# lucidrains/magvit2-pytorch

Hardware: NVIDIA H100
Metric: video-frames/sec tokenize+decode, 17x128x128 bf16 (higher is better)
Workload: dtype bf16

## Files before the change

magvit2_pytorch_b200/csrc/tc_common.cuh:

```cuda
#pragma once
#include "common.cuh"
#include <cuda.h>
#include <mutex>

namespace mv2 {


__device__ __forceinline__ uint32_t smem_u32(const void* p) { return (uint32_t)__cvta_generic_to_shared(p); }

__device__ __forceinline__ void mbar_init(uint32_t bar, uint32_t count) {
  asm volatile("mbarrier.init.shared::cta.b64 [%0], %1;" ::"r"(bar), "r"(count));
}
__device__ __forceinline__ void mbar_expect_tx(uint32_t bar, uint32_t bytes) {
  asm volatile("mbarrier.arrive.expect_tx.shared::cta.b64 _, [%0], %1;" ::"r"(bar), "r"(bytes) : "memory");
}
__device__ __forceinline__ void mbar_wait(uint32_t bar, uint32_t parity) {
  asm volatile(
      "{\n\t"
      ".reg .pred P1;\n\t"
      "WAIT_LOOP:\n\t"
      "mbarrier.try_wait.parity.shared::cta.b64 P1, [%0], %1, 0x989680;\n\t"
      "@P1 bra DONE;\n\t"
      "bra WAIT_LOOP;\n\t"
      "DONE:\n\t"
      "}" ::"r"(bar), "r"(parity) : "memory");
}
__device__ __forceinline__ void fence_barrier_init() { asm volatile("fence.mbarrier_init.release.cluster;" ::: "memory"); }
__device__ __forceinline__ void fence_proxy_async() { asm volatile("fence.proxy.async.shared::cta;" ::: "memory"); }

__device__ __forceinline__ void tma_load_5d(uint32_t dst, const CUtensorMap* map, uint32_t bar, int c0, int c1, int c2,
                                            int c3, int c4) {
  asm volatile(
      "cp.async.bulk.tensor.5d.shared::cluster.global.tile.mbarrier::complete_tx::bytes [%0], [%1, {%3, %4, %5, %6, %7}], [%2];"
      ::"r"(dst), "l"(map), "r"(bar), "r"(c0), "r"(c1), "r"(c2), "r"(c3), "r"(c4) : "memory");
}
__device__ __forceinline__ void tma_load_2d(uint32_t dst, const CUtensorMap* map, uint32_t bar, int c0, int c1) {
  asm volatile(
      "cp.async.bulk.tensor.2d.shared::cluster.global.tile.mbarrier::complete_tx::bytes [%0], [%1, {%3, %4}], [%2];"
      ::"r"(dst), "l"(map), "r"(bar), "r"(c0), "r"(c1) : "memory");
}
__device__ __forceinline__ void tma_load_3d(uint32_t dst, const CUtensorMap* map, uint32_t bar, int c0, int c1, int c2) {
  asm volatile(
      "cp.async.bulk.tensor.3d.shared::cluster.global.tile.mbarrier::complete_tx::bytes [%0], [%1, {%3, %4, %5}], [%2];"
      ::"r"(dst), "l"(map), "r"(bar), "r"(c0), "r"(c1), "r"(c2) : "memory");
}
__device__ __forceinline__ void tma_prefetch_desc(const CUtensorMap* map) {
  asm volatile("prefetch.tensormap [%0];" ::"l"(map) : "memory");
}

__device__ __forceinline__ void wgmma_fence() { asm volatile("wgmma.fence.sync.aligned;" ::: "memory"); }
__device__ __forceinline__ void wgmma_commit() { asm volatile("wgmma.commit_group.sync.aligned;" ::: "memory"); }
__device__ __forceinline__ void wgmma_wait_all() { asm volatile("wgmma.wait_group.sync.aligned 0;" ::: "memory"); }
template <int N> __device__ __forceinline__ void wgmma_wait() { asm volatile("wgmma.wait_group.sync.aligned %0;" ::"n"(N) : "memory"); }

template <int N> __device__ __forceinline__ void setmaxnreg_dec() { asm volatile("setmaxnreg.dec.sync.aligned.u32 %0;" ::"n"(N)); }
template <int N> __device__ __forceinline__ void setmaxnreg_inc() { asm volatile("setmaxnreg.inc.sync.aligned.u32 %0;" ::"n"(N)); }
template <int N> __device__ __forceinline__ void wgmma_bf16(float (&d)[N / 2], uint64_t da, uint64_t db, uint32_t scale_d);
template <> __device__ __forceinline__ void wgmma_bf16<8>(float (&d)[4], uint64_t da, uint64_t db, uint32_t scale_d) {
  asm volatile(
      "{\n\t.reg .pred p;\n\tsetp.ne.b32 p, %6, 0;\n\t"
      "wgmma.mma_async.sync.aligned.m64n8k16.f32.bf16.bf16 {%0, %1, %2, %3}, %4, %5, p, 1, 1, 0, 0;\n\t}"
      : "+f"(d[0]), "+f"(d[1]), "+f"(d[2]), "+f"(d[3])
      : "l"(da), "l"(db), "r"(scale_d));
}
template <> __device__ __forceinline__ void wgmma_bf16<16>(float (&d)[8], uint64_t da, uint64_t db, uint32_t scale_d) {
  asm volatile(
      "{\n\t.reg .pred p;\n\tsetp.ne.b32 p, %10, 0;\n\t"
      "wgmma.mma_async.sync.aligned.m64n16k16.f32.bf16.bf16 {%0, %1, %2, %3, %4, %5, %6, %7}, %8, %9, p, 1, 1, 0, 0;\n\t}"
      : "+f"(d[0]), "+f"(d[1]), "+f"(d[2]), "+f"(d[3]), "+f"(d[4]), "+f"(d[5]), "+f"(d[6]), "+f"(d[7])
      : "l"(da), "l"(db), "r"(scale_d));
}
template <> __device__ __forceinline__ void wgmma_bf16<32>(float (&d)[16], uint64_t da, uint64_t db, uint32_t scale_d) {
  asm volatile(
      "{\n\t.reg .pred p;\n\tsetp.ne.b32 p, %18, 0;\n\t"
      "wgmma.mma_async.sync.aligned.m64n32k16.f32.bf16.bf16 {%0, %1, %2, %3, %4, %5, %6, %7, %8, %9, %10, %11, %12, %13, %14, %15}, %16, %17, p, 1, 1, 0, 0;\n\t}"
      : "+f"(d[0]), "+f"(d[1]), "+f"(d[2]), "+f"(d[3]), "+f"(d[4]), "+f"(d[5]), "+f"(d[6]), "+f"(d[7]), "+f"(d[8]), "+f"(d[9]), "+f"(d[10]), "+f"(d[11]), "+f"(d[12]), "+f"(d[13]), "+f"(d[14]), "+f"(d[15])
      : "l"(da), "l"(db), "r"(scale_d));
}
template <> __device__ __forceinline__ void wgmma_bf16<64>(float (&d)[32], uint64_t da, uint64_t db, uint32_t scale_d) {
  asm volatile(
      "{\n\t.reg .pred p;\n\tsetp.ne.b32 p, %34, 0;\n\t"
      "wgmma.mma_async.sync.aligned.m64n64k16.f32.bf16.bf16 {%0, %1, %2, %3, %4, %5, %6, %7, %8, %9, %10, %11, %12, %13, %14, %15, %16, %17, %18, %19, %20, %21, %22, %23, %24, %25, %26, %27, %28, %29, %30, %31}, %32, %33, p, 1, 1, 0, 0;\n\t}"
      : "+f"(d[0]), "+f"(d[1]), "+f"(d[2]), "+f"(d[3]), "+f"(d[4]), "+f"(d[5]), "+f"(d[6]), "+f"(d[7]), "+f"(d[8]), "+f"(d[9]), "+f"(d[10]), "+f"(d[11]), "+f"(d[12]), "+f"(d[13]), "+f"(d[14]), "+f"(d[15]), "+f"(d[16]), "+f"(d[17]), "+f"(d[18]), "+f"(d[19]), "+f"(d[20]), "+f"(d[21]), "+f"(d[22]), "+f"(d[23]), "+f"(d[24]), "+f"(d[25]), "+f"(d[26]), "+f"(d[27]), "+f"(d[28]), "+f"(d[29]), "+f"(d[30]), "+f"(d[31])
      : "l"(da), "l"(db), "r"(scale_d));
}
template <> __device__ __forceinline__ void wgmma_bf16<128>(float (&d)[64], uint64_t da, uint64_t db, uint32_t scale_d) {
  asm volatile(
      "{\n\t.reg .pred p;\n\tsetp.ne.b32 p, %66, 0;\n\t"
      "wgmma.mma_async.sync.aligned.m64n128k16.f32.bf16.bf16 {%0, %1, %2, %3, %4, %5, %6, %7, %8, %9, %10, %11, %12, %13, %14, %15, %16, %17, %18, %19, %20, %21, %22, %23, %24, %25, %26, %27, %28, %29, %30, %31, %32, %33, %34, %35, %36, %37, %38, %39, %40, %41, %42, %43, %44, %45, %46, %47, %48, %49, %50, %51, %52, %53, %54, %55, %56, %57, %58, %59, %60, %61, %62, %63}, %64, %65, p, 1, 1, 0, 0;\n\t}"
      : "+f"(d[0]), "+f"(d[1]), "+f"(d[2]), "+f"(d[3]), "+f"(d[4]), "+f"(d[5]), "+f"(d[6]), "+f"(d[7]), "+f"(d[8]), "+f"(d[9]), "+f"(d[10]), "+f"(d[11]), "+f"(d[12]), "+f"(d[13]), "+f"(d[14]), "+f"(d[15]), "+f"(d[16]), "+f"(d[17]), "+f"(d[18]), "+f"(d[19]), "+f"(d[20]), "+f"(d[21]), "+f"(d[22]), "+f"(d[23]), "+f"(d[24]), "+f"(d[25]), "+f"(d[26]), "+f"(d[27]), "+f"(d[28]), "+f"(d[29]), "+f"(d[30]), "+f"(d[31]), "+f"(d[32]), "+f"(d[33]), "+f"(d[34]), "+f"(d[35]), "+f"(d[36]), "+f"(d[37]), "+f"(d[38]), "+f"(d[39]), "+f"(d[40]), "+f"(d[41]), "+f"(d[42]), "+f"(d[43]), "+f"(d[44]), "+f"(d[45]), "+f"(d[46]), "+f"(d[47]), "+f"(d[48]), "+f"(d[49]), "+f"(d[50]), "+f"(d[51]), "+f"(d[52]), "+f"(d[53]), "+f"(d[54]), "+f"(d[55]), "+f"(d[56]), "+f"(d[57]), "+f"(d[58]), "+f"(d[59]), "+f"(d[60]), "+f"(d[61]), "+f"(d[62]), "+f"(d[63])
      : "l"(da), "l"(db), "r"(scale_d));
}

__host__ __device__ __forceinline__ uint64_t gmma_desc_hi(uint32_t sbo, uint32_t row_bytes) {
  const uint64_t layout = row_bytes == 128 ? 1 : (row_bytes == 64 ? 2 : 3);
  return ((uint64_t)1 << 16) | ((uint64_t)(sbo >> 4) << 32) | (layout << 62);
}
__device__ __forceinline__ uint32_t desc_lo(uint32_t saddr) { return (saddr & 0x3FFFF) >> 4; }

template <int N> __device__ __forceinline__ void stage_acc(const float (&d)[N / 2], float* stg, int t) {
  const int r = 16 * (t >> 5) + ((t & 31) >> 2), c = 2 * (t & 3);
#pragma unroll
  for (int j = 0; j < N / 8; ++j) {
    *reinterpret_cast<float2*>(stg + r * (N + 4) + 8 * j + c) = make_float2(d[4 * j], d[4 * j + 1]);
    *reinterpret_cast<float2*>(stg + (r + 8) * (N + 4) + 8 * j + c) = make_float2(d[4 * j + 2], d[4 * j + 3]);
  }
}
__device__ __forceinline__ void load_row32(const float* src, int ncols, uint32_t (&r)[32]) {
#pragma unroll
  for (int g = 0; g < 8; ++g) {
    if (g * 4 >= ncols) break;
    const float4 v = *reinterpret_cast<const float4*>(src + 4 * g);
    r[4 * g] = __float_as_uint(v.x); r[4 * g + 1] = __float_as_uint(v.y);
    r[4 * g + 2] = __float_as_uint(v.z); r[4 * g + 3] = __float_as_uint(v.w);
  }
}
__device__ __forceinline__ void named_bar_sync(uint32_t id, uint32_t nthreads) {
  asm volatile("bar.sync %0, %1;" ::"r"(id), "r"(nthreads) : "memory");
}
__device__ __forceinline__ void mbar_arrive(uint32_t bar) {
  asm volatile("mbarrier.arrive.shared::cta.b64 _, [%0];" ::"r"(bar) : "memory");
}

__device__ __forceinline__ uint32_t pack_bf16x2(float a, float b) {
  __nv_bfloat162 v = __floats2bfloat162_rn(a, b);
  return *reinterpret_cast<uint32_t*>(&v);
}



struct TcEpi {
  const float* bias;
  const __nv_bfloat16* res;
  __nv_bfloat16* y;
  int act, shuffle, mode;
  int Co;
  int To, Ho, Wo;
  int out_cf;
  const float* oscale;
};

__device__ __forceinline__ void store8_bf16(__nv_bfloat16* dst, const float (&v)[8]) {
  uint4 o;
  o.x = pack_bf16x2(v[0], v[1]); o.y = pack_bf16x2(v[2], v[3]);
  o.z = pack_bf16x2(v[4], v[5]); o.w = pack_bf16x2(v[6], v[7]);
  *reinterpret_cast<uint4*>(dst) = o;
}

enum { EPI_PLAIN = 0, EPI_GEGLU = 1, EPI_SHUFFLE = 2, EPI_RAGGED = 3, EPI_PLAIN_RES = 4, EPI_FUSED_RU = 5, EPI_SHUFFLE_ST = 6,
       EPI_DOWN_SPACE = 7 };

__device__ __forceinline__ float ex2_approx(float x) {
  float y;
  asm("ex2.approx.ftz.f32 %0, %1;" : "=f"(y) : "f"(x));
  return y;
}
__device__ __forceinline__ float rcp_approx(float x) {
  float y;
  asm("rcp.approx.ftz.f32 %0, %1;" : "=f"(y) : "f"(x));
  return y;
}
__device__ __forceinline__ float erf_fast(float x) {
  const float ax = fabsf(x);
  const float t = rcp_approx(fmaf(0.3275911f, ax, 1.f));
  float p = fmaf(1.061405429f, t, -1.453152027f);
  p = fmaf(p, t, 1.421413741f);
  p = fmaf(p, t, -0.284496736f);
  p = fmaf(p, t, 0.254829592f);
  const float e = ex2_approx(-1.4426950408889634f * ax * ax);
  return copysignf(fmaf(-p * t, e, 1.f), x);
}

__device__ __forceinline__ float gelu_fast(float g) {
  const float ag = fabsf(g);
  const float t = rcp_approx(fmaf(0.3275911f * 0.70710678118654752440f, ag, 1.f));
  float p = fmaf(0.5f * 1.061405429f, t, 0.5f * -1.453152027f);
  p = fmaf(p, t, 0.5f * 1.421413741f);
  p = fmaf(p, t, 0.5f * -0.284496736f);
  p = fmaf(p, t, 0.5f * 0.254829592f);
  const float e = ex2_approx((g * g) * (-0.5f * 1.4426950408889634f));
  const float q = (p * t) * e;
  return fmaf(-ag, q, fmaxf(g, 0.f));
}

template <int ACT>
__device__ __forceinline__ float act_ct(float x, bool relu = false) {
  if (ACT == MV2_ACT_ELU) {
    const float e = ex2_approx(x * 1.4426950408889634f) - 1.f;
    return x > 0.f ? x : e;
  }
  if (ACT == MV2_ACT_SILU) return x * rcp_approx(1.f + ex2_approx(-1.4426950408889634f * x));
  if (ACT == MV2_ACT_LEAKY_RELU) return x > 0.f ? x : (relu ? 0.f * x : 0.1f * x);
  return x;
}

template <int MODE, int ACT>
__device__ __forceinline__ void epi_chunk32_t(const TcEpi& e, const uint32_t (&r)[32], int ncols, int n, const float* sb,
                                              int b, int to, int ho, int wo, int64_t row_base, bool relu = false) {
  if (MODE == EPI_GEGLU) {
    const int I = e.Co >> 1;
    const int64_t pos = (((int64_t)b * e.To + to) * e.Ho + ho) * e.Wo + wo;
#pragma unroll
    for (int g = 0; g < 2; ++g) {
      if (g * 16 >= ncols || n + g * 16 >= e.Co) break;
      float v[8];
#pragma unroll
      for (int q = 0; q < 8; ++q) {
        const float xv = __uint_as_float(r[g * 16 + q]) + sb[g * 16 + q];
        const float gt = __uint_as_float(r[g * 16 + 8 + q]) + sb[g * 16 + 8 + q];
        v[q] = gelu_fast(gt) * xv;
      }
      store8_bf16(e.y + pos * I + ((n + g * 16) >> 1), v);
    }
    return;
  }
  const int cy = MODE == EPI_SHUFFLE ? (e.shuffle == MV2_SHUFFLE_SPACE ? (e.Co >> 2) : (e.Co >> 1)) : e.Co;
  const bool vec_ok = (cy & 7) == 0;
#pragma unroll
  for (int g = 0; g < 4; ++g) {
    const int ng = n + g * 8;
    if (g * 8 >= ncols || ng >= e.Co) break;
    float v[8];
    {
      const float4 b0 = *reinterpret_cast<const float4*>(sb + g * 8), b1 = *reinterpret_cast<const float4*>(sb + g * 8 + 4);
      const float bb[8] = {b0.x, b0.y, b0.z, b0.w, b1.x, b1.y, b1.z, b1.w};
      if (MODE != EPI_SHUFFLE && e.oscale) {
#pragma unroll
        for (int q = 0; q < 8; ++q) {
          const float os = ng + q < e.Co ? e.oscale[(int64_t)b * e.Co + ng + q] : 0.f;
          v[q] = act_ct<ACT>(__uint_as_float(r[g * 8 + q]) * os + bb[q], relu);
        }
      } else
#pragma unroll
      for (int q = 0; q < 8; ++q) v[q] = act_ct<ACT>(__uint_as_float(r[g * 8 + q]) + bb[q], relu);
    }
    int64_t off;
    if (MODE == EPI_SHUFFLE) {
      const int qd = ng / cy, c = ng - qd * cy;
      if (e.shuffle == MV2_SHUFFLE_SPACE) {
        const int p1 = qd >> 1, p2 = qd & 1;
        off = ((((int64_t)b * e.To + to) * (2 * e.Ho) + (2 * ho + p1)) * (2 * e.Wo) + (2 * wo + p2)) * cy + c;
      } else {
        off = ((((int64_t)b * (2 * e.To) + (2 * to + qd)) * e.Ho + ho) * e.Wo + wo) * cy + c;
      }
    } else {
      off = row_base + ng;
    }
    const float rscale = e.mode == 2 ? 0.70710678118654752440f : 1.f;
    if (vec_ok && ng + 8 <= e.Co) {
      if (e.res) {
        const uint4 rv = *reinterpret_cast<const uint4*>(e.res + off);
        const __nv_bfloat162* rb = reinterpret_cast<const __nv_bfloat162*>(&rv);
#pragma unroll
        for (int q = 0; q < 4; ++q) {
          const float2 f = __bfloat1622float2(rb[q]);
          v[2 * q] = (v[2 * q] + f.x) * rscale;
          v[2 * q + 1] = (v[2 * q + 1] + f.y) * rscale;
        }
      }
      store8_bf16(e.y + off, v);
    } else {
      if (MODE == EPI_RAGGED && e.out_cf) {
        const int64_t plane = (int64_t)e.Ho * e.Wo;
        const int64_t o0 = ((int64_t)b * e.Co * e.To + to) * plane + (int64_t)ho * e.Wo + wo;
        for (int q = 0; q < 8 && ng + q < e.Co; ++q) e.y[o0 + (int64_t)(ng + q) * e.To * plane] = __float2bfloat16_rn(v[q]);
      } else
      for (int q = 0; q < 8 && ng + q < e.Co; ++q) {
        float x = v[q];
        if (e.res) x = (x + __bfloat162float(e.res[off + q])) * rscale;
        e.y[off + q] = __float2bfloat16_rn(x);
      }
    }
  }
}

template <int ACT>
__device__ __forceinline__ void epi_pack32_t(const uint32_t (&r)[32], const float* sb, uint32_t (&pk)[16], bool relu = false) {
#pragma unroll
  for (int g = 0; g < 8; ++g) {
    const float4 b = *reinterpret_cast<const float4*>(sb + g * 4);
    pk[2 * g] = pack_bf16x2(act_ct<ACT>(__uint_as_float(r[4 * g]) + b.x, relu), act_ct<ACT>(__uint_as_float(r[4 * g + 1]) + b.y, relu));
    pk[2 * g + 1] = pack_bf16x2(act_ct<ACT>(__uint_as_float(r[4 * g + 2]) + b.z, relu), act_ct<ACT>(__uint_as_float(r[4 * g + 3]) + b.w, relu));
  }
}
template <int ACT>
__device__ __forceinline__ void epi_act32_t(uint32_t (&r)[32], const float* sb, bool relu = false) {
#pragma unroll
  for (int g = 0; g < 8; ++g) {
    const float4 b = *reinterpret_cast<const float4*>(sb + g * 4);
    r[4 * g] = __float_as_uint(act_ct<ACT>(__uint_as_float(r[4 * g]) + b.x, relu));
    r[4 * g + 1] = __float_as_uint(act_ct<ACT>(__uint_as_float(r[4 * g + 1]) + b.y, relu));
    r[4 * g + 2] = __float_as_uint(act_ct<ACT>(__uint_as_float(r[4 * g + 2]) + b.z, relu));
    r[4 * g + 3] = __float_as_uint(act_ct<ACT>(__uint_as_float(r[4 * g + 3]) + b.w, relu));
  }
}
__device__ __forceinline__ void epi_act32(int act, uint32_t (&r)[32], const float* sb) {
  if (act == MV2_ACT_ELU) epi_act32_t<MV2_ACT_ELU>(r, sb);
  else if (act == MV2_ACT_SILU) epi_act32_t<MV2_ACT_SILU>(r, sb);
  else if (act == MV2_ACT_LEAKY_RELU || act == MV2_ACT_RELU) epi_act32_t<MV2_ACT_LEAKY_RELU>(r, sb, act == MV2_ACT_RELU);
  else epi_act32_t<MV2_ACT_NONE>(r, sb);
}
__device__ __forceinline__ void epi_pack32(int act, const uint32_t (&r)[32], const float* sb, uint32_t (&pk)[16]) {
  if (act == MV2_ACT_ELU) epi_pack32_t<MV2_ACT_ELU>(r, sb, pk);
  else if (act == MV2_ACT_SILU) epi_pack32_t<MV2_ACT_SILU>(r, sb, pk);
  else if (act == MV2_ACT_LEAKY_RELU || act == MV2_ACT_RELU) epi_pack32_t<MV2_ACT_LEAKY_RELU>(r, sb, pk, act == MV2_ACT_RELU);
  else epi_pack32_t<MV2_ACT_NONE>(r, sb, pk);
}

template <int MODE>
__device__ __forceinline__ void epi_chunk32(const TcEpi& e, const uint32_t (&r)[32], int ncols, int n, const float* sb,
                                            int b, int to, int ho, int wo, int64_t row_base) {
  if (MODE == EPI_GEGLU) { epi_chunk32_t<EPI_GEGLU, MV2_ACT_NONE>(e, r, ncols, n, sb, b, to, ho, wo, row_base); return; }
  if (e.act == MV2_ACT_ELU) epi_chunk32_t<MODE, MV2_ACT_ELU>(e, r, ncols, n, sb, b, to, ho, wo, row_base);
  else if (e.act == MV2_ACT_SILU) epi_chunk32_t<MODE, MV2_ACT_SILU>(e, r, ncols, n, sb, b, to, ho, wo, row_base);
  else if (e.act == MV2_ACT_LEAKY_RELU || e.act == MV2_ACT_RELU)
    epi_chunk32_t<MODE, MV2_ACT_LEAKY_RELU>(e, r, ncols, n, sb, b, to, ho, wo, row_base, e.act == MV2_ACT_RELU);
  else epi_chunk32_t<MODE, MV2_ACT_NONE>(e, r, ncols, n, sb, b, to, ho, wo, row_base);
}

typedef CUresult (*EncodeTiledFn)(CUtensorMap*, CUtensorMapDataType, cuuint32_t, void*, const cuuint64_t*,
                                  const cuuint64_t*, const cuuint32_t*, const cuuint32_t*, CUtensorMapInterleave,
                                  CUtensorMapSwizzle, CUtensorMapL2promotion, CUtensorMapFloatOOBfill);

static inline EncodeTiledFn get_encode_fn() {
  static EncodeTiledFn fn = nullptr;
  static std::once_flag once;
  std::call_once(once, [] {
    void* f = nullptr;
    cudaDriverEntryPointQueryResult q;
    if (cudaGetDriverEntryPoint("cuTensorMapEncodeTiled", &f, cudaEnableDefault, &q) == cudaSuccess &&
        q == cudaDriverEntryPointSuccess)
      fn = (EncodeTiledFn)f;
  });
  return fn;
}

static inline CUtensorMapSwizzle swizzle_of_row(int row_bytes) {
  return row_bytes == 128 ? CU_TENSOR_MAP_SWIZZLE_128B : (row_bytes == 64 ? CU_TENSOR_MAP_SWIZZLE_64B : CU_TENSOR_MAP_SWIZZLE_32B);
}

static inline int encode_bf16_map(CUtensorMap* map, int rank, const void* base, const cuuint64_t* dims,
                                  const cuuint64_t* strides, const cuuint32_t* box, CUtensorMapSwizzle swz, const char* what) {
  const EncodeTiledFn enc = get_encode_fn();
  if (!enc) { set_error("cuTensorMapEncodeTiled entry point unavailable"); return MV2_E_CUDA; }
  const cuuint32_t es[5] = {1, 1, 1, 1, 1};
  const CUresult r = enc(map, CU_TENSOR_MAP_DATA_TYPE_BFLOAT16, (cuuint32_t)rank, const_cast<void*>(base), dims, strides, box, es,
                         CU_TENSOR_MAP_INTERLEAVE_NONE, swz, CU_TENSOR_MAP_L2_PROMOTION_L2_256B, CU_TENSOR_MAP_FLOAT_OOB_FILL_NONE);
  if (r != CUDA_SUCCESS) { set_error("cuTensorMapEncodeTiled(%s) failed: %d", what, (int)r); return MV2_E_CUDA; }
  return MV2_OK;
}

static inline TcEpi tc_epi_of(const mv2_tc_conv_args* a) {
  TcEpi e = {};
  e.bias = a->bias; e.res = (const __nv_bfloat16*)a->res; e.y = (__nv_bfloat16*)a->y;
  e.act = a->act; e.shuffle = a->shuffle; e.mode = a->epi_mode; e.Co = a->Co;
  e.To = a->To; e.Ho = a->Ho; e.Wo = a->Wo; e.out_cf = a->out_layout == 1; e.oscale = a->oscale;
  return e;
}

static inline int pow2_ceil(int v) { int r = 1; while (r < v) r <<= 1; return r; }
static inline int floor_div(int a, int b) { int q = a / b; if ((a % b != 0) && ((a < 0) != (b < 0))) --q; return q; }


}
```

magvit2_pytorch_b200/csrc/tc_slab.cu:

```cuda
#include "common.cuh"
#include "tc_common.cuh"
#include <cuda.h>
#include <algorithm>
#include <type_traits>
#include <mutex>
#include <map>
#include <vector>
#include <string.h>

namespace mv2 {

struct alignas(64) SlabParams {
  CUtensorMap amap;
  CUtensorMap hmap;
  CUtensorMap wmap;
  CUtensorMap wmap2;
  int kt, kh, kw, pt, ph, pw;
  int st;
  int hist_T;
  int Ci, kchunks, row_bytes;
  int B, T, H, W, Co;
  int mw, pitch, slab_h, slab_bytes, slab_stride;
  int bn, n_tiles_n, tiles_w, tiles_h, total_tiles;
  int slab_stages, w_stages;
  int tpw;
  TcEpi epi;
  CUtensorMap w1map;
  const float* bias1;
  const float* se_wk;
  float se_bk;
  float* se_ws;
  CUtensorMap amap_odd;
  int dn_e_off;
  int dn_aoff[6];
  int dn_lower;
  int h_stride;
};

__host__ __device__ __forceinline__ void slab_frame_of(const SlabParams& p, int slot, int& b, int& t) {
  const int ptc = p.pt > 0 ? (p.pt + p.st - 1) / p.st : 0;
  const int n_cheap = ptc < p.T ? ptc : p.T, n_full = p.T - n_cheap;
  const int full_slots = p.B * n_full;
  if (slot < full_slots) { b = slot / n_full; t = n_cheap + slot - b * n_full; }
  else { const int r = slot - full_slots; const int level = r / p.B; b = r - level * p.B; t = n_cheap - 1 - level; }
}
__host__ __device__ __forceinline__ int slab_tile_of_cta(const SlabParams& p, int k, int cta, int grid) {
  const int tile = k * grid + ((k & 1) ? grid - 1 - cta : cta);
  return tile < p.total_tiles ? tile : -1;
}
__device__ __forceinline__ int slab_tile_of(const SlabParams& p, int k) { return slab_tile_of_cta(p, k, blockIdx.x, gridDim.x); }

struct TileCoord { int b, t, h0, w0, n0; };
__host__ __device__ __forceinline__ TileCoord decode_tile(const SlabParams& p, int tile) {
  TileCoord c;
  const int nt = tile % p.n_tiles_n; tile /= p.n_tiles_n;
  const int tw = tile % p.tiles_w; tile /= p.tiles_w;
  const int th = tile % p.tiles_h; tile /= p.tiles_h;
  slab_frame_of(p, tile, c.b, c.t);
  c.h0 = th * 16;
  c.w0 = tw * 8 * p.mw;
  c.n0 = nt * p.bn;
  return c;
}

struct SlabSmem { uint32_t sbias, stage0, lpart, accstg, hbuf, end; };
__host__ __device__ __forceinline__ SlabSmem slab_smem_layout(const SlabParams& p, uint32_t bar0, bool fused) {
  SlabSmem m;
  m.sbias = (bar0 + 8 * (2 * p.slab_stages + 2 * p.w_stages) + 15) & ~15u;
  m.stage0 = m.sbias + (uint32_t)(p.n_tiles_n * p.bn) * 4 * (fused ? 3 : 1);
  m.lpart = m.stage0 + (fused ? 0 : 8 * 2048);
  m.accstg = m.lpart + (fused ? 2048 : 0);
  m.hbuf = m.accstg + 2u * p.mw * 64 * (p.bn + 4) * 4;
  if (fused) m.hbuf = (m.hbuf + 1023u) & ~1023u;
  m.end = m.hbuf + (fused ? (uint32_t)p.h_stride : 0);
  return m;
}

constexpr int SLAB_PRODUCER_REGS = 40, SLAB_CONSUMER_REGS = 232;
template <int MODE, int BN>
__global__ void __launch_bounds__(384, 1) tc_slab_kernel(const __grid_constant__ SlabParams p) {
  constexpr int MWMAX = BN >= 32 ? 128 / BN : 4;
  constexpr int KC1 = BN >= 64 ? BN / 64 : 1;
  extern __shared__ uint8_t smem_raw[];
  const uint32_t smem_base = (smem_u32(smem_raw) + 1023u) & ~1023u;
  const int warp = threadIdx.x >> 5, lane = threadIdx.x & 31;
  const uint32_t row_bytes = p.row_bytes;
  const uint32_t bk = row_bytes >> 1;
  const uint32_t w_tile = p.bn * row_bytes;
  const uint32_t w_bytes = w_tile * p.tpw;
  const uint32_t slab0 = smem_base;
  const uint32_t wst0 = smem_base + p.slab_stages * p.slab_stride;
  const uint32_t bar0 = wst0 + p.w_stages * w_bytes;
  const uint32_t slab_full = bar0, slab_empty = slab_full + 8 * p.slab_stages;
  const uint32_t w_full = slab_empty + 8 * p.slab_stages, w_empty = w_full + 8 * p.w_stages;
  const SlabSmem L = slab_smem_layout(p, bar0, MODE == EPI_FUSED_RU);
  auto gen = [&](uint32_t u) { return smem_raw + (u - smem_u32(smem_raw)); };
  float* sbias = reinterpret_cast<float*>(gen(L.sbias));
  const uint32_t nbias = (uint32_t)(p.n_tiles_n * p.bn);
  const uint32_t stage0 = L.stage0;

  if (threadIdx.x == 0) {
    for (int s = 0; s < p.slab_stages; ++s) { mbar_init(slab_full + 8 * s, 1); mbar_init(slab_empty + 8 * s, 8); }
    for (int s = 0; s < p.w_stages; ++s) { mbar_init(w_full + 8 * s, 1); mbar_init(w_empty + 8 * s, 8); }
    fence_barrier_init();
  }
  if (warp == 0 && lane == 0) {
    tma_prefetch_desc(&p.amap);
    if (MODE == EPI_DOWN_SPACE) tma_prefetch_desc(&p.amap_odd);
    else if (p.hist_T > 0) tma_prefetch_desc(&p.hmap);
  }
  if (warp == 2 && lane == 0) {
    tma_prefetch_desc(&p.wmap); tma_prefetch_desc(&p.wmap2);
    if (MODE == EPI_FUSED_RU) tma_prefetch_desc(&p.w1map);
  }
  if (warp >= 4) {
    const int nb = p.n_tiles_n * p.bn;
    for (int i = threadIdx.x - 128; i < nb; i += 256) sbias[i] = (p.epi.bias && i < p.Co) ? p.epi.bias[i] : 0.f;
    if (MODE == EPI_FUSED_RU)
      for (int i = threadIdx.x - 128; i < nb; i += 256) {
        sbias[nb + i] = (p.bias1 && i < p.Co) ? p.bias1[i] : 0.f;
        sbias[2 * nb + i] = i < p.Co ? p.se_wk[i] : 0.f;
      }
  }
  __syncthreads();
  pdl_wait();
  pdl_launch_dependents();

  const int taps2d = p.kh * p.kw;

  if (warp < 4) {
    setmaxnreg_dec<SLAB_PRODUCER_REGS>();
    if (warp == 0) {
      if (MODE == EPI_DOWN_SPACE) {
        if (lane == 0) {
          uint32_t s = 0, ph = 0;
          for (int tk = 0, tile; (tile = slab_tile_of(p, tk)) >= 0; ++tk) {
            const TileCoord c = decode_tile(p, tile);
            for (int kc = 0; kc < p.kchunks; ++kc) {
              mbar_wait(slab_empty + 8 * s, ph ^ 1);
              mbar_expect_tx(slab_full + 8 * s, p.slab_bytes);
              tma_load_5d(slab0 + s * p.slab_stride, &p.amap_odd, slab_full + 8 * s, kc * bk, c.w0 - 1, c.h0 - 1, c.t, c.b);
              tma_load_5d(slab0 + s * p.slab_stride + p.dn_e_off, &p.amap, slab_full + 8 * s, kc * bk, c.w0 - 1, c.h0, c.t, c.b);
              if (++s == (uint32_t)p.slab_stages) { s = 0; ph ^= 1; }
            }
          }
        }
      } else
      if (lane == 0) {
        uint32_t s = 0, ph = 0;
        for (int tk = 0, tile; (tile = slab_tile_of(p, tk)) >= 0; ++tk) {
          const TileCoord c = decode_tile(p, tile);
          const int dt0 = max(0, p.pt - c.t * p.st - p.hist_T);
          for (int dt = dt0; dt < p.kt; ++dt)
            for (int kc = 0; kc < p.kchunks; ++kc) {
              mbar_wait(slab_empty + 8 * s, ph ^ 1);
              mbar_expect_tx(slab_full + 8 * s, p.slab_bytes);
              const int ti = c.t * p.st + dt - p.pt;
              tma_load_5d(slab0 + s * p.slab_stride, ti >= 0 ? &p.amap : &p.hmap, slab_full + 8 * s, kc * bk, c.w0 - p.pw,
                          c.h0 - p.ph, ti >= 0 ? ti : ti + p.hist_T, c.b);
              if (++s == (uint32_t)p.slab_stages) { s = 0; ph ^= 1; }
            }
        }
      }
    } else if (warp == 2) {
      if (MODE == EPI_DOWN_SPACE) {
        if (lane == 0) {
          uint32_t s = 0, ph = 0;
          const int C2 = p.Ci;
          for (int tk = 0, tile; (tile = slab_tile_of(p, tk)) >= 0; ++tk) {
            const TileCoord c = decode_tile(p, tile);
            for (int kc = 0; kc < p.kchunks; ++kc)
              for (int tap = kc < p.dn_lower ? 1 : 0; tap < 6; tap += kc < p.dn_lower ? 2 : 1) {
                mbar_wait(w_empty + 8 * s, ph ^ 1);
                mbar_expect_tx(w_full + 8 * s, w_tile);
                tma_load_2d(wst0 + s * w_bytes, &p.wmap2, w_full + 8 * s, tap * C2 + kc * (int)bk, c.n0);
                if (++s == (uint32_t)p.w_stages) { s = 0; ph ^= 1; }
              }
          }
        }
      } else
      if (lane == 0) {
        uint32_t s = 0, ph = 0;
        for (int tk = 0, tile; (tile = slab_tile_of(p, tk)) >= 0; ++tk) {
          const TileCoord c = decode_tile(p, tile);
          const int dt0 = max(0, p.pt - c.t * p.st - p.hist_T);
          for (int dt = dt0; dt < p.kt; ++dt)
            for (int kc = 0; kc < p.kchunks; ++kc)
              for (int tp = 0; tp < taps2d; tp += p.tpw) {
                mbar_wait(w_empty + 8 * s, ph ^ 1);
                mbar_expect_tx(w_full + 8 * s, w_bytes);
                if (p.tpw == 1) tma_load_2d(wst0 + s * w_bytes, &p.wmap2, w_full + 8 * s, (dt * taps2d + tp) * p.Ci + kc * bk, c.n0);
                else tma_load_3d(wst0 + s * w_bytes, &p.wmap, w_full + 8 * s, kc * bk, c.n0, dt * taps2d + tp);
                if (++s == (uint32_t)p.w_stages) { s = 0; ph ^= 1; }
              }
          if (MODE == EPI_FUSED_RU)
            for (int kc2 = 0; kc2 < KC1; ++kc2) {
              mbar_wait(w_empty + 8 * s, ph ^ 1);
              mbar_expect_tx(w_full + 8 * s, w_tile);
              tma_load_2d(wst0 + s * w_bytes, &p.w1map, w_full + 8 * s, kc2 * (int)bk, 0);
              if (++s == (uint32_t)p.w_stages) { s = 0; ph ^= 1; }
            }
        }
      }
    }
  } else {
    setmaxnreg_inc<SLAB_CONSUMER_REGS>();
    const int wg = (warp - 4) >> 2, wq = warp & 3, tid = threadIdx.x & 127;
    const int sub = 2 * wg + (wq & 1), half = wq >> 1, ew = sub + 4 * half;
    const int row = sub * 32 + lane;
    const int lh = row >> 3, lw = row & 7;
    float* stg = reinterpret_cast<float*>(gen(L.accstg)) + (size_t)wg * p.mw * 64 * (BN + 4);
    const uint32_t wg_bar = 5 + wg;
    const uint32_t sbo = (uint32_t)p.pitch * row_bytes;
    const uint64_t a_hi = gmma_desc_hi(sbo, row_bytes);
    const uint64_t b_hi = gmma_desc_hi(8 * row_bytes, row_bytes);
    const bool k4 = bk == 64;
    const uint32_t a_row = row_bytes >> 4;
    const uint32_t a_wg = (uint32_t)wg * 8 * (sbo >> 4);
    const uint32_t a_next_dh = (uint32_t)(p.pitch - p.kw + 1) * a_row;
    const uint32_t a_mtile = 8 * a_row;
    const uint32_t w_tile16 = w_tile >> 4, w_stage16 = w_bytes >> 4;
    const uint32_t b_lo0 = desc_lo(wst0);
    uint32_t s_idx = 0, s_par = 0;
    uint32_t w_idx = 0, w_par = 0, b_lo = b_lo0;
    uint32_t ecount = 0;
    float acc[MWMAX][BN / 2];
    auto mainloop = [&](const TileCoord& c, auto mw_c, auto k4_c) {
      constexpr int MW = decltype(mw_c)::value;
      constexpr bool K4 = decltype(k4_c)::value;
      constexpr uint32_t NONE = ~0u;
      uint32_t accum = 0, pend_w = NONE, pend_s = NONE;
      auto release_pending = [&]() {
        __syncwarp();
        if (lane == 0) {
          if (pend_w != NONE) mbar_arrive(w_empty + 8 * pend_w);
          if (pend_s != NONE) mbar_arrive(slab_empty + 8 * pend_s);
        }
      };
      auto retire_previous = [&](uint32_t w_last, uint32_t s_last) {
        wgmma_wait<1>();
        release_pending();
        pend_w = w_last; pend_s = s_last;
      };
      auto next_w_stage = [&]() {
        if (++w_idx == (uint32_t)p.w_stages) { w_idx = 0; w_par ^= 1; b_lo = b_lo0; } else { b_lo += w_stage16; }
      };
      if (MODE == EPI_DOWN_SPACE) {
        for (int kc = 0; kc < p.kchunks; ++kc) {
          mbar_wait(slab_full + 8 * s_idx, s_par);
          const uint32_t a_base = desc_lo(slab0 + s_idx * p.slab_stride) + a_wg;
          const int t0 = kc < p.dn_lower ? 1 : 0, tstep = kc < p.dn_lower ? 2 : 1;
          for (int tap = t0; tap < 6; tap += tstep) {
            mbar_wait(w_full + 8 * w_idx, w_par);
            wgmma_fence();
            const uint64_t bd = b_hi | (uint64_t)b_lo;
#pragma unroll
            for (int j = 0; j < MW; ++j) {
              const uint64_t ad = a_hi | (uint64_t)(a_base + (uint32_t)p.dn_aoff[tap] + j * a_mtile);
              wgmma_bf16<BN>(acc[j], ad, bd, accum);
              wgmma_bf16<BN>(acc[j], ad + 2, bd + 2, 1u);
              wgmma_bf16<BN>(acc[j], ad + 4, bd + 4, 1u);
              wgmma_bf16<BN>(acc[j], ad + 6, bd + 6, 1u);
            }
            wgmma_commit();
            retire_previous(w_idx, tap + tstep >= 6 ? s_idx : NONE);
            accum = 1;
            next_w_stage();
          }
          if (++s_idx == (uint32_t)p.slab_stages) { s_idx = 0; s_par ^= 1; }
        }
      } else {
        const int dt0 = max(0, p.pt - c.t * p.st - p.hist_T);
        for (int dt = dt0; dt < p.kt; ++dt)
          for (int kc = 0; kc < p.kchunks; ++kc) {
            mbar_wait(slab_full + 8 * s_idx, s_par);
            uint32_t a_lo = desc_lo(slab0 + s_idx * p.slab_stride) + a_wg;
            int dw = 0;
            for (int tp0 = 0; tp0 < taps2d; tp0 += p.tpw) {
              mbar_wait(w_full + 8 * w_idx, w_par);
              const bool slab_last = tp0 + p.tpw >= taps2d;
              uint32_t b_cur = b_lo;
              for (int u = 0; u < p.tpw; ++u) {
                wgmma_fence();
                const uint64_t bd = b_hi | (uint64_t)b_cur;
#pragma unroll
                for (int j = 0; j < MW; ++j) {
                  const uint64_t ad = a_hi | (uint64_t)(a_lo + j * a_mtile);
                  wgmma_bf16<BN>(acc[j], ad, bd, accum);
                  wgmma_bf16<BN>(acc[j], ad + 2, bd + 2, 1u);
                  if (K4) {
                    wgmma_bf16<BN>(acc[j], ad + 4, bd + 4, 1u);
                    wgmma_bf16<BN>(acc[j], ad + 6, bd + 6, 1u);
                  }
                }
                wgmma_commit();
                const bool w_last = u == p.tpw - 1;
                retire_previous(w_last ? w_idx : NONE, w_last && slab_last ? s_idx : NONE);
                accum = 1;
                b_cur += w_tile16;
                if (++dw == p.kw) { dw = 0; a_lo += a_next_dh; } else { a_lo += a_row; }
              }
              next_w_stage();
            }
            if (++s_idx == (uint32_t)p.slab_stages) { s_idx = 0; s_par ^= 1; }
          }
      }
      wgmma_wait<0>();
      release_pending();
    };
    auto mainloop_k = [&](const TileCoord& c, auto mw_c) {
      if (MODE != EPI_FUSED_RU && MODE != EPI_DOWN_SPACE && !k4) mainloop(c, mw_c, std::false_type());
      else mainloop(c, mw_c, std::true_type());
    };
    for (int tk = 0, tile; (tile = slab_tile_of(p, tk)) >= 0; ++tk) {
      const TileCoord c = decode_tile(p, tile);
      if (MWMAX >= 4 && p.mw == 4) mainloop_k(c, std::integral_constant<int, (MWMAX >= 4 ? 4 : 1)>());
      else if (MWMAX >= 2 && p.mw == 2) mainloop_k(c, std::integral_constant<int, (MWMAX >= 2 ? 2 : 1)>());
      else mainloop_k(c, std::integral_constant<int, 1>());
      named_bar_sync(wg_bar, 128);
#pragma unroll
      for (int j = 0; j < MWMAX; ++j) {
        if (j >= p.mw) break;
        stage_acc<BN>(acc[j], stg + j * 64 * (BN + 4), tid);
      }
      named_bar_sync(wg_bar, 128);
      const int h = c.h0 + lh;
      if (MODE == EPI_FUSED_RU) {
        const float* sb1 = sbias + nbias;
        const float* swk = sbias + 2 * nbias;
        float* lpart = reinterpret_cast<float*>(gen(L.lpart));
        const int64_t kstride = (int64_t)p.W * p.Co;
        const uint32_t wsw = (lane >> 1) & 3;
        const int rl = lane >> 2, piece = lane & 3;
        const int h20 = c.h0 + sub * 4;
        const int recs_per_frame = p.tiles_h * p.tiles_w * 4;
        float* rec = p.se_ws + ((int64_t)(c.b * p.T + c.t) * recs_per_frame + ((c.h0 >> 4) * p.tiles_w + c.w0 / (8 * p.mw)) * 4 + sub) * (p.Co + 2);
        float run_m = -INFINITY, run_s = 0.f, run_acc[2][8];
#pragma unroll
        for (int q = 0; q < 2; ++q)
#pragma unroll
          for (int i = 0; i < 8; ++i) run_acc[q][i] = 0.f;
        const uint64_t h_hi = gmma_desc_hi(1024, 128);
        const uint32_t h_lo = desc_lo(L.hbuf) + (uint32_t)wg * ((64 * 128) >> 4);
        uint32_t w1_slot[KC1], w1_par[KC1], w1_lo[KC1];
#pragma unroll
        for (int kc2 = 0; kc2 < KC1; ++kc2) {
          w1_slot[kc2] = w_idx; w1_par[kc2] = w_par; w1_lo[kc2] = b_lo;
          if (++w_idx == (uint32_t)p.w_stages) { w_idx = 0; w_par ^= 1; b_lo = b_lo0; } else { b_lo += w_stage16; }
        }
        for (int j = 0; j < p.mw; ++j) {
          const float* srow = stg + (j * 64 + row - 64 * wg) * (BN + 4);
          const uint32_t stg2 = smem_u32(stg + (j * 64 + (sub & 1) * 32) * (BN + 4)) + (uint32_t)half * 2048;
          const uint32_t wr = stg2 + lane * 64, rd = stg2 + rl * 64;
          const uint32_t hb = L.hbuf + (uint32_t)row * 128;
          for (int c0 = half * 32; c0 < p.bn; c0 += 64) {
            uint32_t r[32], pk[16];
            load_row32(srow + c0, 32, r);
            epi_pack32_t<MV2_ACT_ELU>(r, sbias + c0, pk);
            const uint32_t hrow = hb + (uint32_t)(c0 >> 6) * 16384;
            const uint32_t p0 = (uint32_t)(c0 & 63) >> 3;
#pragma unroll
            for (int g = 0; g < 4; ++g)
              asm volatile("st.shared.v4.b32 [%0], {%1, %2, %3, %4};" ::"r"(hrow + (((p0 + g) ^ ((uint32_t)row & 7u)) << 4)),
                           "r"(pk[4 * g]), "r"(pk[4 * g + 1]), "r"(pk[4 * g + 2]), "r"(pk[4 * g + 3]) : "memory");
          }
          fence_proxy_async();
          named_bar_sync(wg_bar, 128);
#pragma unroll
          for (int kc2 = 0; kc2 < KC1; ++kc2) mbar_wait(w_full + 8 * w1_slot[kc2], w1_par[kc2]);
          wgmma_fence();
#pragma unroll
          for (int kc2 = 0; kc2 < KC1; ++kc2) {
            const uint64_t ad = h_hi | (uint64_t)(h_lo + kc2 * (16384 >> 4)), bd = h_hi | (uint64_t)w1_lo[kc2];
            wgmma_bf16<BN>(acc[0], ad, bd, kc2 > 0 ? 1u : 0u);
            wgmma_bf16<BN>(acc[0], ad + 2, bd + 2, 1u);
            wgmma_bf16<BN>(acc[0], ad + 4, bd + 4, 1u);
            wgmma_bf16<BN>(acc[0], ad + 6, bd + 6, 1u);
          }
          wgmma_commit();
          wgmma_wait<0>();
          if (j == p.mw - 1) {
            __syncwarp();
            if (lane == 0)
#pragma unroll
              for (int kc2 = 0; kc2 < KC1; ++kc2) mbar_arrive(w_empty + 8 * w1_slot[kc2]);
          }
          stage_acc<BN>(acc[0], stg + j * 64 * (BN + 4), tid);
          named_bar_sync(wg_bar, 128);
          const int w = c.w0 + 8 * j + lw;
          const bool row_ok = h < p.H && w < p.W;
          uint32_t pk2[2][16];
          float lp = 0.f;
#pragma unroll
          for (int q = 0; q < 2; ++q) {
            const int c0 = half * 32 + 64 * q;
            if (c0 < p.bn) {
              uint32_t r[32];
              load_row32(srow + c0, 32, r);
              epi_pack32_t<MV2_ACT_ELU>(r, sb1 + c0, pk2[q]);
#pragma unroll
              for (int i = 0; i < 16; i += 2) {
                const float4 wv = *reinterpret_cast<const float4*>(swk + c0 + 2 * i);
                lp = fmaf(__uint_as_float(pk2[q][i] << 16), wv.x, lp);
                lp = fmaf(__uint_as_float(pk2[q][i] & 0xffff0000u), wv.y, lp);
                lp = fmaf(__uint_as_float(pk2[q][i + 1] << 16), wv.z, lp);
                lp = fmaf(__uint_as_float(pk2[q][i + 1] & 0xffff0000u), wv.w, lp);
              }
            }
          }
          float* lpb = lpart + (ecount & 1u) * 256;
          ++ecount;
          lpb[ew * 32 + lane] = lp;
          asm volatile("bar.sync %0, 64;" ::"r"(1 + sub) : "memory");
          float lg = lpb[sub * 32 + lane] + lpb[(sub + 4) * 32 + lane] + p.se_bk;
          lg = row_ok ? lg : -INFINITY;
          const float mx = warp_max(lg);
          const float ev = lg > -INFINITY ? ex2_approx((lg - mx) * 1.4426950408889634f) : 0.f;
          const float es = warp_sum(ev);
          float e4[4];
#pragma unroll
          for (int k = 0; k < 4; ++k) e4[k] = __shfl_sync(0xffffffffu, ev, 8 * k + rl);
          const float new_m = fmaxf(run_m, mx);
          const float ca = run_m > -INFINITY ? ex2_approx((run_m - new_m) * 1.4426950408889634f) : 0.f;
          const float cb = mx > -INFINITY ? ex2_approx((mx - new_m) * 1.4426950408889634f) : 0.f;
          run_s = fmaf(run_s, ca, es * cb);
          run_m = new_m;
          const int w2 = c.w0 + 8 * j + rl;
          const int64_t row0 = ((((int64_t)c.b * p.T + c.t) * p.H + h20) * p.W + w2) * p.Co + piece * 8;
          const int kmax = w2 < p.W ? p.H - h20 : 0;
#pragma unroll
          for (int q = 0; q < 2; ++q) {
            const int c0 = half * 32 + 64 * q;
            if (c0 < p.bn) {
#pragma unroll
              for (int g = 0; g < 4; ++g)
                asm volatile("st.shared.v4.b32 [%0], {%1, %2, %3, %4};" ::"r"(wr + ((g ^ wsw) << 4)), "r"(pk2[q][4 * g]),
                             "r"(pk2[q][4 * g + 1]), "r"(pk2[q][4 * g + 2]), "r"(pk2[q][4 * g + 3]) : "memory");
              __syncwarp();
              __nv_bfloat16* yp = p.epi.y + row0 + c0;
              float t[8];
#pragma unroll
              for (int i = 0; i < 8; ++i) t[i] = 0.f;
#pragma unroll
              for (int k = 0; k < 4; ++k) {
                uint4 v;
                asm volatile("ld.shared.v4.b32 {%0, %1, %2, %3}, [%4];" : "=r"(v.x), "=r"(v.y), "=r"(v.z), "=r"(v.w)
                             : "r"(rd + k * 512 + ((piece ^ (((8 * k + rl) >> 1) & 3)) << 4)));
                if (k < kmax) *reinterpret_cast<uint4*>(yp + k * kstride) = v;
                const uint32_t vv[4] = {v.x, v.y, v.z, v.w};
#pragma unroll
                for (int i = 0; i < 4; ++i) {
                  t[2 * i] = fmaf(e4[k], __uint_as_float(vv[i] << 16), t[2 * i]);
                  t[2 * i + 1] = fmaf(e4[k], __uint_as_float(vv[i] & 0xffff0000u), t[2 * i + 1]);
                }
              }
              __syncwarp();
#pragma unroll
              for (int i = 0; i < 8; ++i) {
                t[i] += __shfl_xor_sync(0xffffffffu, t[i], 4);
                t[i] += __shfl_xor_sync(0xffffffffu, t[i], 8);
                t[i] += __shfl_xor_sync(0xffffffffu, t[i], 16);
              }
#pragma unroll
              for (int i = 0; i < 8; ++i) run_acc[q][i] = fmaf(run_acc[q][i], ca, t[i] * cb);
            }
          }
        }
        if (half == 0 && lane == 0) { rec[0] = run_m; rec[1] = run_s; }
        if (rl == 0) {
#pragma unroll
          for (int q = 0; q < 2; ++q) {
            const int c0 = half * 32 + 64 * q;
            if (c0 < p.bn) {
              float2* dst = reinterpret_cast<float2*>(rec + 2 + c0 + piece * 8);
              dst[0] = make_float2(run_acc[q][0], run_acc[q][1]); dst[1] = make_float2(run_acc[q][2], run_acc[q][3]);
              dst[2] = make_float2(run_acc[q][4], run_acc[q][5]); dst[3] = make_float2(run_acc[q][6], run_acc[q][7]);
            }
          }
        }
      } else
      for (int j = 0; j < p.mw; ++j) {
        const int w = c.w0 + 8 * j + lw;
        const bool row_ok = h < p.H && w < p.W;
        const float* srow = stg + (j * 64 + row - 64 * wg) * (BN + 4);
        const int64_t row_base = ((((int64_t)c.b * p.T + c.t) * p.H + h) * p.W + w) * p.Co;
        if (MODE == EPI_PLAIN || MODE == EPI_PLAIN_RES || MODE == EPI_SHUFFLE_ST || MODE == EPI_DOWN_SPACE) {
          const uint32_t stg = stage0 + (uint32_t)ew * 2048;
          const uint32_t wr = stg + lane * 64, wsw = (lane >> 1) & 3;
          const int rl = lane >> 2, piece = lane & 3;
          const int w2 = c.w0 + 8 * j + rl;
          const uint32_t rd = stg + rl * 64;
          const int h20 = c.h0 + sub * 4;
          const int64_t row0 = ((((int64_t)c.b * p.T + c.t) * p.H + h20) * p.W + w2) * p.Co + c.n0 + piece * 8;
          const int64_t kstride = (int64_t)p.W * p.Co;
          const int kmax = w2 < p.W ? p.H - h20 : 0;
          for (int c0 = ((j + half) & 1) * 32; c0 < p.bn; c0 += 64) {
            uint32_t r[32], pk[16];
            uint4 rv[4];
            if (MODE == EPI_PLAIN_RES) {
              const __nv_bfloat16* rr = p.epi.res + row_base + c.n0 + c0;
#pragma unroll
              for (int g = 0; g < 4; ++g)
                rv[g] = (row_ok && c.n0 + c0 + g * 8 < p.Co && c0 + g * 8 < p.bn) ? *reinterpret_cast<const uint4*>(rr + g * 8) : make_uint4(0, 0, 0, 0);
            }
            load_row32(srow + c0, 32, r);
            if ((MODE == EPI_PLAIN || MODE == EPI_PLAIN_RES) && p.epi.oscale) {
              const float* os = p.epi.oscale + (int64_t)c.b * p.Co + c.n0 + c0;
#pragma unroll
              for (int i = 0; i < 32; ++i) r[i] = __float_as_uint(__uint_as_float(r[i]) * (c.n0 + c0 + i < p.Co ? os[i] : 0.f));
            }
            if (MODE == EPI_PLAIN_RES) {
              epi_act32(p.epi.act, r, sbias + c.n0 + c0);
              const float rs = p.epi.mode == 2 ? 0.70710678118654752440f : 1.f;
#pragma unroll
              for (int g = 0; g < 4; ++g) {
                const uint32_t w4[4] = {rv[g].x, rv[g].y, rv[g].z, rv[g].w};
#pragma unroll
                for (int q = 0; q < 4; ++q)
                  pk[4 * g + q] = pack_bf16x2((__uint_as_float(r[8 * g + 2 * q]) + __uint_as_float(w4[q] << 16)) * rs,
                                              (__uint_as_float(r[8 * g + 2 * q + 1]) + __uint_as_float(w4[q] & 0xffff0000u)) * rs);
              }
            } else
            epi_pack32(p.epi.act, r, sbias + c.n0 + c0, pk);
#pragma unroll
            for (int g = 0; g < 4; ++g)
              asm volatile("st.shared.v4.b32 [%0], {%1, %2, %3, %4};" ::"r"(wr + ((g ^ wsw) << 4)), "r"(pk[4 * g]),
                           "r"(pk[4 * g + 1]), "r"(pk[4 * g + 2]), "r"(pk[4 * g + 3]) : "memory");
            __syncwarp();
            const bool col_ok = c.n0 + c0 + piece * 8 < p.Co && c0 + piece * 8 < p.bn;
            const int klim = col_ok ? kmax : 0;
            __nv_bfloat16* yp;
            int64_t ks;
            if (MODE == EPI_SHUFFLE_ST) {
              const int n = c.n0 + c0;
              if (p.epi.shuffle == MV2_SHUFFLE_SPACE) {
                const int cy = p.Co >> 2, qd = n / cy, cb = n - qd * cy;
                yp = p.epi.y + ((((int64_t)c.b * p.T + c.t) * (2 * p.H) + (2 * h20 + (qd >> 1))) * (2 * p.W) + (2 * w2 + (qd & 1))) * cy + cb + piece * 8;
                ks = (int64_t)4 * p.W * cy;
              } else {
                const int cy = p.Co >> 1, qd = n / cy, cb = n - qd * cy;
                yp = p.epi.y + ((((int64_t)c.b * (2 * p.T) + (2 * c.t + qd)) * p.H + h20) * p.W + w2) * cy + cb + piece * 8;
                ks = (int64_t)p.W * cy;
              }
            } else {
              yp = p.epi.y + row0 + c0;
              ks = kstride;
            }
#pragma unroll
            for (int k = 0; k < 4; ++k) {
              uint4 v;
              asm volatile("ld.shared.v4.b32 {%0, %1, %2, %3}, [%4];" : "=r"(v.x), "=r"(v.y), "=r"(v.z), "=r"(v.w)
                           : "r"(rd + k * 512 + ((piece ^ (((8 * k + rl) >> 1) & 3)) << 4)));
              if (k < klim) *reinterpret_cast<uint4*>(yp + k * ks) = v;
            }
            __syncwarp();
          }
        } else {
          for (int c0 = ((j + half) & 1) * 32; c0 < p.bn; c0 += 64) {
            uint32_t r[32];
            load_row32(srow + c0, BN < 32 ? BN : 32, r);
            if (row_ok) epi_chunk32<MODE>(p.epi, r, min(32, p.bn - c0), c.n0 + c0, sbias + c.n0 + c0, c.b, c.t, h, w, row_base);
          }
        }
      }
    }
  }
}

}

using namespace mv2;

static bool slab_narrow(const mv2_tc_conv_args* a) { return a->out_layout == 1 && a->Co <= 16 && a->kw > 3; }

extern "C" int mv2_tc_slab_supported(const mv2_tc_conv_args* a) {
  if (!a) return 0;
  if (a->sh != 1 || a->sw != 1) return 0;
  if (a->st != 1) {
    if (a->st != 2 || a->out_layout != 0 || a->epi_mode != 0 || a->shuffle != MV2_SHUFFLE_NONE) return 0;
    if (a->To != (a->Ti + a->pt - a->kt) / a->st + 1 || a->To < 1) return 0;
  }
  if (a->Ci % 32 != 0 || a->Co > 4096) return 0;
  if (a->oscale && (a->epi_mode != 0 || a->shuffle != MV2_SHUFFLE_NONE)) return 0;
  if (a->epi_mode == 1 && (a->Co % 64 != 0 || a->shuffle != MV2_SHUFFLE_NONE || a->res)) return 0;
  if (a->epi_mode == 2 && (!a->res || a->shuffle != MV2_SHUFFLE_NONE)) return 0;
  if (a->epi_mode < 0 || a->epi_mode > 2) return 0;
  if (a->Co % 32 != 0 && a->Co > 32) return 0;
  if (a->Ci % 64 != 0 && a->kw != 1) return 0;
  if (a->res && a->Co % 8 != 0) return 0;
  if (a->shuffle != MV2_SHUFFLE_NONE && ((a->shuffle == MV2_SHUFFLE_SPACE ? a->Co / 4 : a->Co / 2) % 8 != 0 || a->Co % 32 != 0)) return 0;
  if (a->kh > 7 || a->kw > (slab_narrow(a) ? 7 : 3) || a->kt > 8) return 0;
  if (a->Ho != a->Hi || a->Wo != a->Wi) return 0;
  if (a->out_layout == 1) {
    if (a->Co % 8 == 0 || a->res || a->shuffle != MV2_SHUFFLE_NONE || a->epi_mode != 0) return 0;
    if (a->To > a->Ti || a->To < 1) return 0;
    if (a->pt != a->kt - 1 - (a->Ti - a->To) && a->pt != -(a->Ti - a->To)) return 0;
  } else if (a->out_layout != 0 || (a->st == 1 && a->To != a->Ti)) return 0;
  return 1;
}

static int slab_ring_budget(const SlabParams& p, bool fused) {
  SlabParams q = p;
  q.slab_stages = 3; q.w_stages = 12;
  return 227 * 1024 - 2048 - (int)slab_smem_layout(q, 0, fused).end;
}
static size_t slab_smem_bytes(const SlabParams& p, bool fused) {
  const uint32_t rings = (uint32_t)(p.slab_stages * p.slab_stride + p.w_stages * p.bn * p.row_bytes * p.tpw);
  return 1024 + slab_smem_layout(p, rings, fused).end;
}
static int slab_default_mw(int bn, int Wo) { return bn <= 32 && Wo > 16 ? 4 : (bn <= 64 && Wo > 8 ? 2 : 1); }
static void slab_set_geometry(SlabParams& p, int mw) {
  p.mw = mw;
  p.pitch = 8 * mw + p.kw - 1;
  p.slab_bytes = p.pitch * p.slab_h * p.row_bytes;
  p.slab_stride = (p.slab_bytes + 1023) / 1024 * 1024;
  p.tiles_w = ceil_div(p.W, 8 * mw);
  p.total_tiles = (int)((int64_t)p.B * p.T * p.tiles_h * p.tiles_w * p.n_tiles_n);
}

static int slab_fill_plan(const mv2_tc_conv_args* a, SlabParams& p) {
  memset(&p, 0, sizeof(p));
  p.kt = a->kt; p.kh = a->kh; p.kw = a->kw; p.pt = a->pt; p.ph = a->ph; p.pw = a->pw;
  p.st = a->st;
  p.row_bytes = (a->Ci % 64 == 0) ? 128 : 64;
  p.Ci = a->Ci; p.kchunks = a->Ci / (p.row_bytes / 2);
  p.B = a->B; p.T = a->To; p.H = a->Ho; p.W = a->Wo; p.Co = a->Co;
  p.epi = tc_epi_of(a);

// ... 253 lines not shown
```

Baseline: 5008.

## Swap wgmma operands for BN=64 so weights act as the M dimension

For BN=64 kernels, the wgmma operands are swapped: weights become the A operand (64 output channels as M) and slab pixels become the B operand with N=64 or 128. When mw==2 this replaces two m64n64 MMAs per k-step with one m64n128, and each warpgroup takes a different pixel subtile. The transposed accumulator is staged to shared memory with a new transposed store routine, and when mw==2 the staging buffer is shared across both consumer warpgroups behind a 256-thread barrier. This aims to cut MMA instruction count and improve tensor-core efficiency, at the cost of strided, possibly bank-conflicted smem stores and cross-warpgroup synchronisation.

```diff
diff --git a/magvit2_pytorch_b200/csrc/tc_common.cuh b/magvit2_pytorch_b200/csrc/tc_common.cuh
--- a/magvit2_pytorch_b200/csrc/tc_common.cuh
+++ b/magvit2_pytorch_b200/csrc/tc_common.cuh
@@ -104,6 +104,15 @@
   for (int j = 0; j < N / 8; ++j) {
     *reinterpret_cast<float2*>(stg + r * (N + 4) + 8 * j + c) = make_float2(d[4 * j], d[4 * j + 1]);
     *reinterpret_cast<float2*>(stg + (r + 8) * (N + 4) + 8 * j + c) = make_float2(d[4 * j + 2], d[4 * j + 3]);
+  }
+}
+template <int N> __device__ __forceinline__ void stage_acc_t(const float (&d)[N / 2], float* stg, int t) {
+  const int r = 16 * (t >> 5) + ((t & 31) >> 2), c = 2 * (t & 3);
+#pragma unroll
+  for (int j = 0; j < N / 8; ++j) {
+    float* s = stg + (8 * j + c) * 68 + r;
+    s[0] = d[4 * j]; s[68] = d[4 * j + 1];
+    s[8] = d[4 * j + 2]; s[68 + 8] = d[4 * j + 3];
   }
 }
 __device__ __forceinline__ void load_row32(const float* src, int ncols, uint32_t (&r)[32]) {
diff --git a/magvit2_pytorch_b200/csrc/tc_slab.cu b/magvit2_pytorch_b200/csrc/tc_slab.cu
--- a/magvit2_pytorch_b200/csrc/tc_slab.cu
+++ b/magvit2_pytorch_b200/csrc/tc_slab.cu
@@ -81,6 +81,7 @@
 __global__ void __launch_bounds__(384, 1) tc_slab_kernel(const __grid_constant__ SlabParams p) {
   constexpr int MWMAX = BN >= 32 ? 128 / BN : 4;
   constexpr int KC1 = BN >= 64 ? BN / 64 : 1;
+  constexpr bool SWAP = BN == 64;
   extern __shared__ uint8_t smem_raw[];
   const uint32_t smem_base = (smem_u32(smem_raw) + 1023u) & ~1023u;
   const int warp = threadIdx.x >> 5, lane = threadIdx.x & 31;
@@ -211,6 +212,8 @@
     const int lh = row >> 3, lw = row & 7;
     float* stg = reinterpret_cast<float*>(gen(L.accstg)) + (size_t)wg * p.mw * 64 * (BN + 4);
     const uint32_t wg_bar = 5 + wg;
+    const bool stg_shared = SWAP && p.mw == 2;
+    const uint32_t stg_bar = stg_shared ? 7 : wg_bar, stg_threads = stg_shared ? 256 : 128;
     const uint32_t sbo = (uint32_t)p.pitch * row_bytes;
     const uint64_t a_hi = gmma_desc_hi(sbo, row_bytes);
     const uint64_t b_hi = gmma_desc_hi(8 * row_bytes, row_bytes);
@@ -245,23 +248,41 @@
       auto next_w_stage = [&]() {
         if (++w_idx == (uint32_t)p.w_stages) { w_idx = 0; w_par ^= 1; b_lo = b_lo0; } else { b_lo += w_stage16; }
       };
+      const uint32_t a_off = SWAP && MW == 2 ? (uint32_t)wg * a_mtile : a_wg;
+      auto tap_mma = [&](uint32_t s_lo, uint32_t w_lo, uint32_t scale_d) {
+        const uint64_t wd = b_hi | (uint64_t)w_lo;
+        if constexpr (SWAP) {
+          constexpr int NP = MW == 2 ? 128 : 64;
+          float(&d)[NP / 2] = *reinterpret_cast<float(*)[NP / 2]>(&acc[0][0]);
+          const uint64_t sd = a_hi | (uint64_t)s_lo;
+          wgmma_bf16<NP>(d, wd, sd, scale_d);
+          wgmma_bf16<NP>(d, wd + 2, sd + 2, 1u);
+          if (K4) {
+            wgmma_bf16<NP>(d, wd + 4, sd + 4, 1u);
+            wgmma_bf16<NP>(d, wd + 6, sd + 6, 1u);
+          }
+        } else {
+#pragma unroll
+          for (int j = 0; j < MW; ++j) {
+            const uint64_t ad = a_hi | (uint64_t)(s_lo + j * a_mtile);
+            wgmma_bf16<BN>(acc[j], ad, wd, scale_d);
+            wgmma_bf16<BN>(acc[j], ad + 2, wd + 2, 1u);
+            if (K4) {
+              wgmma_bf16<BN>(acc[j], ad + 4, wd + 4, 1u);
+              wgmma_bf16<BN>(acc[j], ad + 6, wd + 6, 1u);
+            }
+          }
+        }
+      };
       if (MODE == EPI_DOWN_SPACE) {
         for (int kc = 0; kc < p.kchunks; ++kc) {
           mbar_wait(slab_full + 8 * s_idx, s_par);
-          const uint32_t a_base = desc_lo(slab0 + s_idx * p.slab_stride) + a_wg;
+          const uint32_t a_base = desc_lo(slab0 + s_idx * p.slab_stride) + a_off;
           const int t0 = kc < p.dn_lower ? 1 : 0, tstep = kc < p.dn_lower ? 2 : 1;
           for (int tap = t0; tap < 6; tap += tstep) {
             mbar_wait(w_full + 8 * w_idx, w_par);
             wgmma_fence();
-            const uint64_t bd = b_hi | (uint64_t)b_lo;
-#pragma unroll
-            for (int j = 0; j < MW; ++j) {
-              const uint64_t ad = a_hi | (uint64_t)(a_base + (uint32_t)p.dn_aoff[tap] + j * a_mtile);
-              wgmma_bf16<BN>(acc[j], ad, bd, accum);
-              wgmma_bf16<BN>(acc[j], ad + 2, bd + 2, 1u);
-              wgmma_bf16<BN>(acc[j], ad + 4, bd + 4, 1u);
-              wgmma_bf16<BN>(acc[j], ad + 6, bd + 6, 1u);
-            }
+            tap_mma(a_base + (uint32_t)p.dn_aoff[tap], b_lo, accum);
             wgmma_commit();
             retire_previous(w_idx, tap + tstep >= 6 ? s_idx : NONE);
             accum = 1;
@@ -274,7 +295,7 @@
         for (int dt = dt0; dt < p.kt; ++dt)
           for (int kc = 0; kc < p.kchunks; ++kc) {
             mbar_wait(slab_full + 8 * s_idx, s_par);
-            uint32_t a_lo = desc_lo(slab0 + s_idx * p.slab_stride) + a_wg;
+            uint32_t a_lo = desc_lo(slab0 + s_idx * p.slab_stride) + a_off;
             int dw = 0;
             for (int tp0 = 0; tp0 < taps2d; tp0 += p.tpw) {
               mbar_wait(w_full + 8 * w_idx, w_par);
@@ -282,17 +303,7 @@
               uint32_t b_cur = b_lo;
               for (int u = 0; u < p.tpw; ++u) {
                 wgmma_fence();
-                const uint64_t bd = b_hi | (uint64_t)b_cur;
-#pragma unroll
-                for (int j = 0; j < MW; ++j) {
-                  const uint64_t ad = a_hi | (uint64_t)(a_lo + j * a_mtile);
-                  wgmma_bf16<BN>(acc[j], ad, bd, accum);
-                  wgmma_bf16<BN>(acc[j], ad + 2, bd + 2, 1u);
-                  if (K4) {
-                    wgmma_bf16<BN>(acc[j], ad + 4, bd + 4, 1u);
-                    wgmma_bf16<BN>(acc[j], ad + 6, bd + 6, 1u);
-                  }
-                }
+                tap_mma(a_lo, b_cur, accum);
                 wgmma_commit();
                 const bool w_last = u == p.tpw - 1;
                 retire_previous(w_last ? w_idx : NONE, w_last && slab_last ? s_idx : NONE);
@@ -317,13 +328,23 @@
       if (MWMAX >= 4 && p.mw == 4) mainloop_k(c, std::integral_constant<int, (MWMAX >= 4 ? 4 : 1)>());
       else if (MWMAX >= 2 && p.mw == 2) mainloop_k(c, std::integral_constant<int, (MWMAX >= 2 ? 2 : 1)>());
       else mainloop_k(c, std::integral_constant<int, 1>());
-      named_bar_sync(wg_bar, 128);
-#pragma unroll
-      for (int j = 0; j < MWMAX; ++j) {
-        if (j >= p.mw) break;
-        stage_acc<BN>(acc[j], stg + j * 64 * (BN + 4), tid);
+      named_bar_sync(stg_bar, stg_threads);
+      if constexpr (SWAP) {
+        if (stg_shared) {
+          float* const stg_all = reinterpret_cast<float*>(gen(L.accstg));
+          stage_acc_t<64>(acc[0], stg_all + (size_t)wg * 64 * (BN + 4), tid);
+          stage_acc_t<64>(acc[1], stg_all + (size_t)(2 + wg) * 64 * (BN + 4), tid);
+        } else {
+          stage_acc_t<64>(acc[0], stg, tid);
+        }
+      } else {
+#pragma unroll
+        for (int j = 0; j < MWMAX; ++j) {
+          if (j >= p.mw) break;
+          stage_acc<BN>(acc[j], stg + j * 64 * (BN + 4), tid);
+        }
       }
-      named_bar_sync(wg_bar, 128);
+      named_bar_sync(stg_bar, stg_threads);
       const int h = c.h0 + lh;
       if (MODE == EPI_FUSED_RU) {
         const float* sb1 = sbias + nbias;
```

New measurement: 5046, median of 6. No clear change (+0.8%).
